# Nadeem202020/VisionTransformer-Intention-Prediction

Hardware: AMD Instinct MI355X
Metric: BEV samples/sec (fwd+bwd) IntentNetViT at 1/2/4/8 MI355X; attn MFMA util % (higher is better)
Workload: dtype bf16

## Files before the change

### visiontransformer-intention-prediction_amd/csrc/attention.hip

```cpp

#include "attn_common.h"

#include <hip/hip_ext.h>

#include <mutex>
#include <vector>

namespace {

constexpr float TAU = 8.0f;

IVIT_DEV float vmax3(float a, float b, float c) {
  float d;
  asm("v_max3_f32 %0, %1, %2, %3" : "=v"(d) : "v"(a), "v"(b), "v"(c));
  return d;
}

struct FwdLdsOff {
  unsigned k[4], v[2][2];
};
IVIT_DEV FwdLdsOff fwd_lds_off(int lane) {
  FwdLdsOff o;
  const int hl = lane >> 5;
#pragma unroll
  for (int ks = 0; ks < 4; ++ks) o.k[ks] = (unsigned)t_off(lane & 31, 2 * ks + hl);
  const int G = lane >> 4, q = (lane >> 2) & 3, p = lane & 3;
#pragma unroll
  for (int cb = 0; cb < 2; ++cb) {
    const int col = 32 * cb + 16 * (G & 1) + 4 * p;
    const int r0 = 4 * (G >> 1) + q, c = col >> 3, e = (col & 7) * 2;
    o.v[cb][0] = (unsigned)(t_off(r0, c) + e);
    o.v[cb][1] = (unsigned)(t_off(r0 + 8, c) + e);
  }
#pragma unroll
  for (int ks = 0; ks < 4; ++ks) asm volatile("" : "+v"(o.k[ks]));
#pragma unroll
  for (int cb = 0; cb < 2; ++cb) asm volatile("" : "+v"(o.v[cb][0]), "+v"(o.v[cb][1]));
  return o;
}

template <bool MASK>
IVIT_DEV float tile_rowmax(f32x16 (&s)[2], int kbase, int N, int lane) {
  const int hl = lane >> 5;
  float a = NEG_BIG, b = NEG_BIG;
#pragma unroll
  for (int t = 0; t < 2; ++t)
#pragma unroll
    for (int r = 0; r < 16; ++r) {
      if (MASK) {
        const int key = kbase + 32 * t + (r & 3) + 8 * (r >> 2) + 4 * hl;
        if (key >= N) s[t][r] = NEG_BIG;
      }
      if (r & 1) b = fmaxf(b, s[t][r]);
      else a = fmaxf(a, s[t][r]);
    }
  return half_swap_max(fmaxf(a, b));
}

IVIT_DEV void qk_tile_c(const char* kimg, const bf16x8 (&qf)[4], const f32x16& init, f32x16 (&s)[2], int lane) {
  const int hl = lane >> 5;
#pragma unroll
  for (int t = 0; t < 2; ++t) {
#pragma unroll
    for (int ks = 0; ks < 4; ++ks) {
      const bf16x8 ka = *(const bf16x8*)(kimg + t_off(32 * t + (lane & 31), 2 * ks + hl));
      s[t] = __builtin_amdgcn_mfma_f32_32x32x16_bf16(ka, qf[ks], ks == 0 ? init : s[t], 0, 0, 0);
    }
  }
}

IVIT_DEV float fwd_step_fenced6(const char* kimg, const char* vimg, const bf16x8 (&qf)[4], const f32x16 (&cur)[2],
                                f32x16 (&nxt)[2], f32x16& o0, f32x16& o1, f32x16& lacc, const bf16x8& ones,
                                const f32x16& negm, int lane, int kbase, int N, const FwdLdsOff& lo) {
  const int hl = lane >> 5;
  auto kfrag = [&](int i) { return *(const bf16x8*)(kimg + lo.k[i & 3] + 4096 * (i >> 2)); };
  unsigned pw[16];
  auto exw = [&](int w) {
    pw[w] = pk_bf16(fast_exp2(cur[(2 * w) >> 4][(2 * w) & 15]), fast_exp2(cur[(2 * w + 1) >> 4][(2 * w + 1) & 15]));
    asm volatile("" : "+v"(pw[w]));
  };
  auto pfrag = [&](int g) {
    return __builtin_bit_cast(bf16x8, make_uint4(pw[4 * g], pw[4 * g + 1], pw[4 * g + 2], pw[4 * g + 3]));
  };
  bf16x8 ka[8];
  ka[0] = kfrag(0);
  ka[1] = kfrag(1);
#pragma unroll
  for (int i = 0; i < 8; ++i) {
    if (i + 2 < 8) ka[i + 2] = kfrag(i + 2);
    const int t = i >> 2, ks = i & 3;
    nxt[t] = __builtin_amdgcn_mfma_f32_32x32x16_bf16(ka[i], qf[ks], ks == 0 ? negm : nxt[t], 0, 0, 0);
    exw(i);
    __builtin_amdgcn_sched_barrier(0);
  }
  bf16x8 vf[8];
  auto vread = [&](int f) {
    union { s16x4 s[2]; bf16x8 v; } u;
    u.s[0] = ds_tr(vimg + lo.v[f & 1][0] + 2048 * (f >> 1));
    u.s[1] = ds_tr(vimg + lo.v[f & 1][1] + 2048 * (f >> 1));
    vf[f] = u.v;
  };
  vread(0);
  vread(1);
  __builtin_amdgcn_sched_barrier(0);
#pragma unroll
  for (int k = 0; k < 6; ++k) {
    const int g = k / 3, which = k % 3;
    if (k == 0) vread(2);
    if (k == 1) vread(3);
    if (k == 3) vread(4);
    if (k == 4) vread(5);
    if (which == 0) o0 = __builtin_amdgcn_mfma_f32_32x32x16_bf16(vf[2 * g], pfrag(g), o0, 0, 0, 0);
    else if (which == 1) o1 = __builtin_amdgcn_mfma_f32_32x32x16_bf16(vf[2 * g + 1], pfrag(g), o1, 0, 0, 0);
    else lacc = __builtin_amdgcn_mfma_f32_32x32x16_bf16(ones, pfrag(g), lacc, 0, 0, 0);
    exw(8 + k);
    __builtin_amdgcn_sched_barrier(0);
  }
  float a = NEG_BIG, bm = NEG_BIG;
  if (kbase + AK > N) {
#pragma unroll
    for (int t = 0; t < 2; ++t)
#pragma unroll
      for (int r = 0; r < 16; ++r) {
        const int key = kbase + 32 * t + (r & 3) + 8 * (r >> 2) + 4 * hl;
        nxt[t][r] = key >= N ? NEG_BIG : nxt[t][r];
      }
  }
#pragma unroll
  for (int k = 6; k < 12; ++k) {
    const int g = k / 3, which = k % 3;
    if (k == 6) vread(6);
    if (k == 7) vread(7);
    if (which == 0) o0 = __builtin_amdgcn_mfma_f32_32x32x16_bf16(vf[2 * g], pfrag(g), o0, 0, 0, 0);
    else if (which == 1) o1 = __builtin_amdgcn_mfma_f32_32x32x16_bf16(vf[2 * g + 1], pfrag(g), o1, 0, 0, 0);
    else lacc = __builtin_amdgcn_mfma_f32_32x32x16_bf16(ones, pfrag(g), lacc, 0, 0, 0);
    if (k == 6) exw(14);
    if (k == 7) exw(15);
    const int v0 = 6 * (k - 6);
#pragma unroll
    for (int v = v0; v < v0 + 6 && v < 32; v += 2) {
      if ((v >> 1) & 1) bm = vmax3(bm, nxt[v >> 4][v & 15], nxt[v >> 4][(v & 15) + 1]);
      else a = vmax3(a, nxt[v >> 4][v & 15], nxt[v >> 4][(v & 15) + 1]);
    }
    __builtin_amdgcn_sched_barrier(0);
  }
  return half_swap_max(fmaxf(a, bm));
}

template <int W, bool PRE>
__global__ __launch_bounds__(64 * W, 8 / W) void attn_fwd_bf16_v6_kernel(const bf16* __restrict__ qkv, int N, int H,
                                                                        bf16* __restrict__ out,
                                                                        float* __restrict__ lse, float c2) {
  __shared__ __attribute__((aligned(16))) char smem[2][2][8192];
  const int tid = threadIdx.x, lane = tid & 63, hl = lane >> 5;
  const int wv = __builtin_amdgcn_readfirstlane(tid >> 6);
  const int2 bid = attn_block_id();
  const int z = bid.y, b = z / H, h = z - b * H;
  const int D = H * 64;
  const long ld = 3L * D;
  const bf16* Qb = qkv + (long)b * N * ld + h * 64;
  const bf16* Kb = Qb + D;
  const bf16* Vb = Qb + 2 * D;
  const int q = bid.x * (32 * W) + wv * 32 + (lane & 31);
  bf16x8 qf[4];
  load_row_frags(Qb + (long)q * ld, q < N, lane, qf);
  if constexpr (PRE) {
#pragma unroll
    for (int i = 0; i < 4; ++i)
#pragma unroll
      for (int e = 0; e < 8; ++e) qf[i][e] = (bf16)((float)qf[i][e] * c2);
  }
  const int nt = (N + AK - 1) / AK, nfull = N / AK;
  unsigned off[8 / W];
#pragma unroll
  for (int i = 0; i < 8 / W; ++i) off[i] = 2u * dma_off<W>(i, wv, lane, ld);
  auto issue1 = [&](const bf16* base, int kt, char* img) {
    const char* sb = uniform_ptr(base + (long)kt * AK * ld);
#pragma unroll
    for (int i = 0; i < 8 / W; ++i) {
      const int piece = wv * (8 / W) + i;
      unsigned o = off[i];
      if (kt >= nfull) {
        const int row = piece * 8 + (lane >> 3), c = (lane & 7) ^ swz128(row);
        o = 2u * (unsigned)((min(kt * AK + row, N - 1) - kt * AK) * ld + c * 8);
      }
      glds_s<false>(o, sb, img + piece * 1024);
    }
  };
  bf16x8 ones;
#pragma unroll
  for (int j = 0; j < 8; ++j) ones[j] = (bf16)1.0f;

  issue1(Kb, 0, smem[0][0]);
  issue1(Vb, 0, smem[0][1]);
  asm volatile("s_waitcnt vmcnt(0)" ::: "memory");
  __builtin_amdgcn_s_barrier();
  if (nt > 1) issue1(Kb, 1, smem[1][0]);
  if (bid.x * (32 * W) + wv * 32 >= N) {
    for (int j = 0; j < nt; ++j) {
      asm volatile("s_waitcnt vmcnt(0)" ::: "memory");
      __builtin_amdgcn_s_barrier();
      if (j + 2 < nt) issue1(Kb, j + 2, smem[j & 1][0]);
      if (j + 1 < nt) issue1(Vb, j + 1, smem[(j & 1) ^ 1][1]);
    }
    return;
  }
  f32x16 sc[2], sn[2];
  qk_tile_c(smem[0][0], qf, zero16(), sc, lane);
  float m = nfull > 0 ? tile_rowmax<false>(sc, 0, N, lane) : tile_rowmax<true>(sc, 0, N, lane);
#pragma unroll
  for (int t = 0; t < 2; ++t)
#pragma unroll
    for (int r = 0; r < 16; ++r) sc[t][r] -= m;
  f32x16 negm;
#pragma unroll
  for (int r = 0; r < 16; ++r) negm[r] = -m;
  f32x16 o0 = zero16(), o1 = zero16(), lacc = zero16();
  const FwdLdsOff lo = fwd_lds_off(lane);

  auto rescale = [&](float mt, f32x16(&nxt)[2]) {
    const bool moved = mt > TAU;
    if (__any(moved)) {
      const float d = moved ? mt : 0.f;
      const float alpha = fast_exp2(-d);
#pragma unroll
      for (int r = 0; r < 16; ++r) { o0[r] *= alpha; o1[r] *= alpha; }
      lacc[0] *= alpha;
#pragma unroll
      for (int t = 0; t < 2; ++t)
#pragma unroll
        for (int r = 0; r < 16; ++r) nxt[t][r] -= d;
      m += d;
#pragma unroll
      for (int r = 0; r < 16; ++r) asm volatile("v_sub_f32 %0, %0, %1" : "+v"(negm[r]) : "v"(d));
    }
  };
  auto body = [&](auto stage, int j, f32x16(&cur)[2], f32x16(&nxt)[2]) {
    constexpr int S = decltype(stage)::value;
    asm volatile("s_waitcnt vmcnt(0)" ::: "memory");
    __builtin_amdgcn_s_barrier();
    if (j + 2 < nt) issue1(Kb, j + 2, smem[S][0]);
    if (j + 1 < nt) issue1(Vb, j + 1, smem[S ^ 1][1]);
    rescale(fwd_step_fenced6(smem[S ^ 1][0], smem[S][1], qf, cur, nxt, o0, o1, lacc, ones, negm, lane,
                               (j + 1) * AK, N, lo),
              nxt);
  };
  using I0 = std::integral_constant<int, 0>;
  using I1 = std::integral_constant<int, 1>;
  int j = 0;
  for (; j + 1 < nt; j += 2) {
    body(I0{}, j, sc, sn);
    body(I1{}, j + 1, sn, sc);
  }
  if (j < nt) body(I0{}, j, sc, sn);
  const float l = lacc[0];
  const float inv = 1.f / l;
  bf16* orow = out + ((long)b * N + (q < N ? q : 0)) * D + h * 64;
  auto emit = [&](const f32x16& o, int dbase) {
#pragma unroll
    for (int g = 0; g < 4; g += 2) {
      const unsigned e0 = pk_bf16(o[4 * g] * inv, o[4 * g + 1] * inv);
      const unsigned e1 = pk_bf16(o[4 * g + 2] * inv, o[4 * g + 3] * inv);
      const unsigned d0 = pk_bf16(o[4 * g + 4] * inv, o[4 * g + 5] * inv);
      const unsigned d1 = pk_bf16(o[4 * g + 6] * inv, o[4 * g + 7] * inv);
      const auto s0 = __builtin_amdgcn_permlane32_swap(d0, e0, false, false);
      const auto s1 = __builtin_amdgcn_permlane32_swap(d1, e1, false, false);
      if (q < N) *(uint4*)(orow + dbase + 8 * (hl ? g : g + 1)) = make_uint4(s0[0], s1[0], s0[1], s1[1]);
    }
  };
  emit(o0, 0);
  emit(o1, 32);
  if (q < N && hl == 0) lse[(long)z * N + q] = (m + log2f(l)) * 0.69314718055994531f;
}

__global__ void attn_prescale_q_kernel(const bf16* __restrict__ qkv, long rows, int D, float c2,
                                       bf16* __restrict__ q2) {
  const long t = (long)blockIdx.x * blockDim.x + threadIdx.x;
  const int cpr = D / 8;
  if (t >= rows * cpr) return;
  const long r = t / cpr;
  const int c = (int)(t - r * cpr) * 8;
  Pack8 x;
  x.u = *(const uint4*)(qkv + r * 3 * D + c);
#pragma unroll
  for (int e = 0; e < 8; ++e) x.h[e] = (bf16)((float)x.h[e] * c2);
  *(uint4*)(q2 + r * D + c) = x.u;
}


constexpr int BNS = 3;

template <int W>
__global__ __launch_bounds__(64 * W, 8 / W) void attn_bwd_dkv_v4_kernel(const bf16* __restrict__ qkv,
                                                                 const bf16* __restrict__ dout,
                                                                 const float* __restrict__ nlse2p,
                                                                 const float* __restrict__ ndeltap, int N, int Npad,
                                                                 int H, bf16* __restrict__ dqkv, float scale,
                                                                 const bf16* __restrict__ qsrc, int ldq) {
  __shared__ __attribute__((aligned(16))) char smem[BNS][2][8192];
  __shared__ __attribute__((aligned(16))) float srow[BNS][2][AK];
  const int tid = threadIdx.x, lane = tid & 63;
  const int g = lane >> 4, c16 = lane & 15;
  const int wv = __builtin_amdgcn_readfirstlane(tid >> 6);
  const int2 bid = attn_block_id();
  const int z = bid.y, b = z / H, h = z - b * H;
  const int D = H * 64;
  const long ld = 3L * D;
  const bf16* Kb = qkv + (long)b * N * ld + D + h * 64;
  const bf16* Vb = Kb + D;
  const bf16* Qb = qsrc + (long)b * N * ldq + h * 64;
  const bf16* Gb = dout + (long)b * N * D + h * 64;
  const char* Ls = uniform_ptr(nlse2p + (long)z * Npad);
  const char* Ds = uniform_ptr(ndeltap + (long)z * Npad);
  constexpr int PW = 8 / W;
  const int kw = bid.x * (32 * W) + wv * 32;
  bf16x8 kf[2][2], vf[2][2];
#pragma unroll
  for (int j = 0; j < 2; ++j) {
    const int key = kw + 16 * j + c16;
#pragma unroll
    for (int s = 0; s < 2; ++s) {
      Pack8 pk, pv;
      pk.u = key < N ? *(const uint4*)(Kb + (long)key * ld + 32 * s + 8 * g) : make_uint4(0, 0, 0, 0);
      pv.u = key < N ? *(const uint4*)(Vb + (long)key * ld + 32 * s + 8 * g) : make_uint4(0, 0, 0, 0);
      kf[j][s] = pk.v;
      vf[j][s] = pv.v;
    }
  }
#pragma unroll
  for (int j = 0; j < 2; ++j) asm volatile("" ::"v"(kf[j][0]), "v"(kf[j][1]), "v"(vf[j][0]), "v"(vf[j][1]));
  f32x4 dk[2][4], dv[2][4];
#pragma unroll
  for (int j = 0; j < 2; ++j)
#pragma unroll
    for (int e = 0; e < 4; ++e) dk[j][e] = dv[j][e] = f32x4{0.f, 0.f, 0.f, 0.f};
  const int nt = (N + AK - 1) / AK, nfull = N / AK;
  unsigned offq[PW], offg[PW];
#pragma unroll
  for (int i = 0; i < PW; ++i) {
    offq[i] = 2u * dma_off16<W>(i, wv, lane, ldq);
    offg[i] = 2u * dma_off16<W>(i, wv, lane, D);
  }
  auto issue = [&](int qt, int S) {
    char* qimg = smem[S][0];
    char* gimg = smem[S][1];
    const char* qb = uniform_ptr(Qb + (long)qt * AK * ldq);
    const char* gb = uniform_ptr(Gb + (long)qt * AK * D);
#pragma unroll
    for (int i = 0; i < PW; ++i) {
      const int piece = wv * PW + i;
      unsigned oq = offq[i], og = offg[i];
      if (qt >= nfull) {
        const int row = piece * 8 + (lane >> 3), c = (lane & 7) ^ (row & 6);
        const int r = min(qt * AK + row, N - 1) - qt * AK;
        oq = 2u * (unsigned)(r * ldq + c * 8);
        og = 2u * (unsigned)(r * D + c * 8);
      }
      glds_s<false>(oq, qb, qimg + piece * 1024);
      glds_s<false>(og, gb, gimg + piece * 1024);
    }
    if (wv == 0) {
      glds4_s(4u * (lane + qt * AK), Ls, &srow[S][0][0]);
      glds4_s(4u * (lane + qt * AK), Ds, &srow[S][1][0]);
    }
  };
  unsigned ro[2], tro[4];
#pragma unroll
  for (int s = 0; s < 2; ++s) ro[s] = (unsigned)t16_off(c16, 4 * s + g);
  {
    const int q = (lane >> 2) & 3, p = lane & 3;
#pragma unroll
    for (int e = 0; e < 4; ++e) tro[e] = (unsigned)(t16_off(4 * g + q, 2 * e + (p >> 1)) + 8 * (p & 1));
  }
#pragma unroll
  for (int s = 0; s < 2; ++s) asm volatile("" : "+v"(ro[s]));
#pragma unroll
  for (int e = 0; e < 4; ++e) asm volatile("" : "+v"(tro[e]));

  bf16x8 qa[2][2], ga[2][2];
  f32x4 sn[2], dn[2];
  bf16x8 tg[4], tq[4];
  auto read_frag = [&](const char* qimg, const char* gimg, int t, int i, int s) {
    qa[i][s] = *(const bf16x8*)(qimg + ro[s] + 4096 * t + 2048 * i);
    ga[i][s] = *(const bf16x8*)(gimg + ro[s] + 4096 * t + 2048 * i);
  };
  auto read_rows = [&](const float* lr, const float* dr, int t, int i) {
    sn[i] = *(const f32x4*)(lr + 32 * t + 16 * i + 4 * g);
    dn[i] = *(const f32x4*)(dr + 32 * t + 16 * i + 4 * g);
  };
  auto word8 = [&](const unsigned (&w)[4]) { return __builtin_bit_cast(bf16x8, make_uint4(w[0], w[1], w[2], w[3])); };
  auto read_b = [&](const char* qimg, const char* gimg, int t, int e) {
    union { s16x4 s[2]; bf16x8 v; } a, c;
    a.s[0] = ds_tr(gimg + tro[e] + 4096 * t);
    a.s[1] = ds_tr(gimg + tro[e] + 4096 * t + 2048);
    c.s[0] = ds_tr(qimg + tro[e] + 4096 * t);
    c.s[1] = ds_tr(qimg + tro[e] + 4096 * t + 2048);
    tg[e] = a.v;
    tq[e] = c.v;
  };
  float ep0, ep1, et0, et1;
  auto e_sub = [&](const f32x4& S, const f32x4& DP, int hh, int ph, unsigned& wu, unsigned& wd) {
    if (ph == 0) {
      ep0 = fast_exp2(S[2 * hh]);
      asm volatile("" : "+v"(ep0));
    }
    if (ph == 1) {
      ep1 = fast_exp2(S[2 * hh + 1]);
      asm volatile("" : "+v"(ep1));
    }
    if (ph == 2) {
      et0 = ep0 * DP[2 * hh];
      et1 = ep1 * DP[2 * hh + 1];
      asm volatile("" : "+v"(et0), "+v"(et1));
    }
    if (ph == 3) {
      wu = pk_bf16(ep0, ep1);
      wd = pk_bf16(et0, et1);
      asm volatile("" : "+v"(wu), "+v"(wd));
    }
  };
  f32x4 sc1[2], dc1[2];
  unsigned upA[4], udA[4];
  unsigned up1[4], ud1[4];
  auto body = [&](auto sa, auto ta, auto sb, auto tb, auto sn_, auto tn, auto bar, int jn, bool more) {
    constexpr int SA = decltype(sa)::value, TA = decltype(ta)::value, SB = decltype(sb)::value;
    constexpr int TB = decltype(tb)::value, SN = decltype(sn_)::value, TN = decltype(tn)::value;
    constexpr bool BAR = decltype(bar)::value;
    f32x4 s[2][2], dp[2][2];
    unsigned upN[4], udN[4];
#pragma unroll
    for (int m = 0; m < 16; ++m) {
      const int ks = m >> 3, i = (m >> 2) & 1, j = (m >> 1) & 1;
      if ((m & 1) == 0) s[i][j] = mfma16(qa[i][ks], kf[j][ks], ks == 0 ? sn[i] : s[i][j]);
      else dp[i][j] = mfma16(ga[i][ks], vf[j][ks], ks == 0 ? dn[i] : dp[i][j]);
      if (m == 0) read_frag(smem[SA][0], smem[SA][1], TA, 0, 1);
      if (m == 2) read_frag(smem[SA][0], smem[SA][1], TA, 1, 1);
      {
        const int q = m >> 2, ie = q >> 1, hh = q & 1;
        e_sub(sc1[ie], dc1[ie], hh, m & 3, up1[2 * ie + hh], ud1[2 * ie + hh]);
      }
      if (m == 9) read_b(smem[SB][0], smem[SB][1], TB, 0);
      if (m == 12) read_b(smem[SB][0], smem[SB][1], TB, 1);
      __builtin_amdgcn_sched_barrier(0);
    }
    if constexpr (BAR) {
      asm volatile("s_waitcnt vmcnt(0)" ::: "memory");
      __builtin_amdgcn_s_barrier();
      if (jn < nt) issue(jn, jn % BNS);
    }
#pragma unroll
    for (int m = 0; m < 16; ++m) {
      const int e = m >> 2, j = (m >> 1) & 1;
      if (m == 0) read_b(smem[SB][0], smem[SB][1], TB, 2);
      if (m == 2) read_b(smem[SB][0], smem[SB][1], TB, 3);
      if ((m & 1) == 0) dv[j][e] = mfma16(word8(j ? up1 : upA), tg[e], dv[j][e]);
      else dk[j][e] = mfma16(word8(j ? ud1 : udA), tq[e], dk[j][e]);
      {
        const int q = m >> 2, ie = q >> 1, hh = q & 1;
        e_sub(s[ie][0], dp[ie][0], hh, m & 3, upN[2 * ie + hh], udN[2 * ie + hh]);
      }
      if (more) {
        if (m == 5) read_rows(srow[SN][0], srow[SN][1], TN, 0);
        if (m == 7) read_rows(srow[SN][0], srow[SN][1], TN, 1);
        if (m == 9) read_frag(smem[SN][0], smem[SN][1], TN, 0, 0);
        if (m == 11) read_frag(smem[SN][0], smem[SN][1], TN, 1, 0);
      }
      __builtin_amdgcn_sched_barrier(0);
    }
#pragma unroll
    for (int i = 0; i < 2; ++i) {
      sc1[i] = s[i][1];
      dc1[i] = dp[i][1];
    }
#pragma unroll
    for (int w = 0; w < 4; ++w) {
      upA[w] = upN[w];
      udA[w] = udN[w];
    }
  };
  using I0 = std::integral_constant<int, 0>;
  using I1 = std::integral_constant<int, 1>;
  using I2 = std::integral_constant<int, 2>;
  using F = std::false_type;
  using T = std::true_type;

  issue(0, 0);
  if (nt > 1) issue(1, 1);
  {
    uint4* z2 = (uint4*)&smem[2][0][0];
    for (int i = tid; i < 2 * 8192 / 16; i += 64 * W) z2[i] = make_uint4(0, 0, 0, 0);
  }
  asm volatile("s_waitcnt vmcnt(0) lgkmcnt(0)" ::: "memory");
  __builtin_amdgcn_s_barrier();
#pragma unroll
  for (int i = 0; i < 2; ++i) {
    read_rows(srow[0][0], srow[0][1], 0, i);
    read_frag(smem[0][0], smem[0][1], 0, i, 0);
  }
#pragma unroll
  for (int i = 0; i < 2; ++i) {
    sc1[i] = f32x4{NEG_BIG, NEG_BIG, NEG_BIG, NEG_BIG};
    dc1[i] = f32x4{0.f, 0.f, 0.f, 0.f};
  }
#pragma unroll
  for (int w = 0; w < 4; ++w) upA[w] = udA[w] = 0u;
  if (kw >= N) {
    for (int j = 0; j < nt; ++j) {
      asm volatile("s_waitcnt vmcnt(0)" ::: "memory");
      __builtin_amdgcn_s_barrier();
      if (j + 2 < nt) issue(j + 2, (j + 2) % BNS);
    }
    __syncthreads();
    return;
  }
  auto tile = [&](auto st, int j) {
    constexpr int S = decltype(st)::value;
    using SP = std::integral_constant<int, (S + BNS - 1) % BNS>;
    using SNX = std::integral_constant<int, (S + 1) % BNS>;
    using SC = std::integral_constant<int, S>;
    body(SC{}, I0{}, SP{}, I1{}, SC{}, I1{}, F{}, 0, true);
    body(SC{}, I1{}, SC{}, I0{}, SNX{}, I0{}, T{}, j + 2, j + 1 < nt);
  };
  int j = 0;
  for (; j + 3 <= nt; j += 3) {
    tile(I0{}, j);
    tile(I1{}, j + 1);
    tile(I2{}, j + 2);
  }
  if (j < nt) tile(I0{}, j);
  if (j + 1 < nt) tile(I1{}, j + 1);
  {
    const int S = (nt - 1) % BNS;
#pragma unroll
    for (int q = 0; q < 4; ++q)
#pragma unroll
      for (int ph = 0; ph < 4; ++ph) e_sub(sc1[q >> 1], dc1[q >> 1], q & 1, ph, up1[q], ud1[q]);
#pragma unroll
    for (int e = 0; e < 4; ++e) read_b(smem[S][0], smem[S][1], 1, e);
#pragma unroll
    for (int e = 0; e < 4; ++e) {
      dv[0][e] = mfma16(word8(upA), tg[e], dv[0][e]);
      dk[0][e] = mfma16(word8(udA), tq[e], dk[0][e]);
      dv[1][e] = mfma16(word8(up1), tg[e], dv[1][e]);
      dk[1][e] = mfma16(word8(ud1), tq[e], dk[1][e]);
    }
  }
  __syncthreads();
  char* tl = &smem[0][0][0] + wv * 2 * 4608;
  bf16* base = dqkv + (long)b * N * ld + h * 64;
  wave_tile_store(tl, dk, scale, base + D, ld, kw, N, lane);
  wave_tile_store(tl + 4608, dv, 1.0f, base + 2 * D, ld, kw, N, lane);
}

IVIT_DEV void dq16_tile_masked(const char* kimg, const char* vimg, const bf16x8 (&qf)[2][2], const bf16x8 (&gf)[2][2],
                               const f32x4 (&nl)[2], const f32x4 (&nd)[2], f32x4 (&dq)[2][4], int kbase, int N,
                               int lane) {
  const int g = lane >> 4, c16 = lane & 15, q = (lane >> 2) & 3, p = lane & 3;
#pragma unroll
  for (int t = 0; t < 2; ++t) {
    if (kbase + 32 * t >= N) break;
    f32x4 s[2][2], dp[2][2];
#pragma unroll
    for (int j = 0; j < 2; ++j)
#pragma unroll
      for (int i = 0; i < 2; ++i) {
        s[j][i] = nl[i];
        dp[j][i] = nd[i];
#pragma unroll
        for (int ks = 0; ks < 2; ++ks) {
          const bf16x8 ka = *(const bf16x8*)(kimg + t16_off(32 * t + 16 * j + c16, 4 * ks + g));
          const bf16x8 va = *(const bf16x8*)(vimg + t16_off(32 * t + 16 * j + c16, 4 * ks + g));
          s[j][i] = mfma16(ka, qf[i][ks], s[j][i]);
          dp[j][i] = mfma16(va, gf[i][ks], dp[j][i]);
        }
      }
    unsigned w[2][4];
#pragma unroll
    for (int i = 0; i < 2; ++i)
#pragma unroll
      for (int j = 0; j < 2; ++j)
#pragma unroll
        for (int hh = 0; hh < 2; ++hh) {
          float d0 = fast_exp2(s[j][i][2 * hh]) * dp[j][i][2 * hh];
          float d1 = fast_exp2(s[j][i][2 * hh + 1]) * dp[j][i][2 * hh + 1];
          const int key = kbase + 32 * t + 16 * j + 4 * g + 2 * hh;
          if (key >= N) d0 = 0.f;
          if (key + 1 >= N) d1 = 0.f;
          w[i][2 * j + hh] = pk_bf16(d0, d1);
        }
#pragma unroll
    for (int e = 0; e < 4; ++e) {
      const int off = t16_off(32 * t + 4 * g + q, 2 * e + (p >> 1)) + 8 * (p & 1);
      union { s16x4 s[2]; bf16x8 v; } u;
      u.s[0] = ds_tr(kimg + off);
      u.s[1] = ds_tr(kimg + off + 2048);
#pragma unroll
      for (int i = 0; i < 2; ++i)
        dq[i][e] = mfma16(__builtin_bit_cast(bf16x8, make_uint4(w[i][0], w[i][1], w[i][2], w[i][3])), u.v, dq[i][e]);
    }
  }
}

template <int W>
__global__ __launch_bounds__(64 * W, 8 / W) void attn_bwd_dq_v4_kernel(const bf16* __restrict__ qkv,
                                                                const bf16* __restrict__ dout,
                                                                float* __restrict__ nlse2p,
                                                                float* __restrict__ ndeltap, int N, int Npad, int H,
                                                                bf16* __restrict__ dqkv, float scale,
                                                                const bf16* __restrict__ out,
                                                                const float* __restrict__ lse,
                                                                const bf16* __restrict__ qsrc, int ldq) {
  __shared__ __attribute__((aligned(16))) char smem[BNS][2][8192];
  const int tid = threadIdx.x, lane = tid & 63;
  const int g = lane >> 4, c16 = lane & 15;
  const int wv = __builtin_amdgcn_readfirstlane(tid >> 6);
  const int2 bid = attn_block_id();
  const int z = bid.y, b = z / H, h = z - b * H;
  const int D = H * 64;
  const long ld = 3L * D;
  const bf16* Kb = qkv + (long)b * N * ld + D + h * 64;
  const bf16* Vb = Kb + D;
  const bf16* Qb = qsrc + (long)b * N * ldq + h * 64;
  constexpr int PW = 8 / W;
  const int qw = bid.x * (32 * W) + wv * 32;
  bf16x8 qf[2][2], gf[2][2];
  f32x4 nl[2], nd[2];
#pragma unroll
  for (int i = 0; i < 2; ++i) {
    const int q = qw + 16 * i + c16;
    const bool qv = q < N;
    bf16x8 of[2];
#pragma unroll
    for (int s = 0; s < 2; ++s) {
      Pack8 pq, pg, po;
      const long orow = ((long)b * N + q) * D + h * 64 + 32 * s + 8 * g;
      pq.u = qv ? *(const uint4*)(Qb + (long)q * ldq + 32 * s + 8 * g) : make_uint4(0, 0, 0, 0);
      pg.u = qv ? *(const uint4*)(dout + orow) : make_uint4(0, 0, 0, 0);
      po.u = qv ? *(const uint4*)(out + orow) : make_uint4(0, 0, 0, 0);
      qf[i][s] = pq.v;
      gf[i][s] = pg.v;
      of[s] = po.v;
    }
    float d = 0.f;
#pragma unroll
    for (int s = 0; s < 2; ++s)
#pragma unroll
      for (int e = 0; e < 8; ++e) d = fmaf((float)of[s][e], (float)gf[i][s][e], d);
    d += __shfl_xor(d, 16, 64);
    d += __shfl_xor(d, 32, 64);
    const float lse2 = qv ? lse[(long)z * N + q] * LOG2E : 1e30f;
    const float dlt = qv ? d : 0.f;
    if (g == 0 && q < Npad) {
      nlse2p[(long)z * Npad + q] = -lse2;
      ndeltap[(long)z * Npad + q] = -dlt;
    }
    nl[i] = f32x4{-lse2, -lse2, -lse2, -lse2};
    nd[i] = f32x4{-dlt, -dlt, -dlt, -dlt};
  }
  f32x4 dq[2][4];
#pragma unroll
  for (int i = 0; i < 2; ++i)
#pragma unroll
    for (int e = 0; e < 4; ++e) dq[i][e] = f32x4{0.f, 0.f, 0.f, 0.f};
  const int nt = (N + AK - 1) / AK, nfull = N / AK;
  unsigned off[PW];
#pragma unroll
  for (int i = 0; i < PW; ++i) off[i] = 2u * dma_off16<W>(i, wv, lane, ld);
  auto issue = [&](int kt, int S) {
    char* kimg = smem[S][0];
    char* vimg = smem[S][1];
    const char* kb = uniform_ptr(Kb + (long)kt * AK * ld);
    const char* vb = uniform_ptr(Vb + (long)kt * AK * ld);
#pragma unroll
    for (int i = 0; i < PW; ++i) {
      const int piece = wv * PW + i;
      unsigned o = off[i];
      if (kt >= nfull) {
        const int row = piece * 8 + (lane >> 3), c = (lane & 7) ^ (row & 6);
        o = 2u * (unsigned)((min(kt * AK + row, N - 1) - kt * AK) * ld + c * 8);
      }
      glds_s<false>(o, kb, kimg + piece * 1024);
      glds_s<false>(o, vb, vimg + piece * 1024);
    }
  };
  issue(0, 0);
  if (nt > 1) issue(1, 1);
  {
    uint4* z2 = (uint4*)&smem[2][0][0];
    for (int i = tid; i < 2 * 8192 / 16; i += 64 * W) z2[i] = make_uint4(0, 0, 0, 0);
  }
  asm volatile("s_waitcnt vmcnt(0) lgkmcnt(0)" ::: "memory");
  __builtin_amdgcn_s_barrier();

  if (qw >= N) {
    for (int j = 0; j < nfull; ++j) {
      asm volatile("s_waitcnt vmcnt(0)" ::: "memory");
      __builtin_amdgcn_s_barrier();
      if (j + 2 < nt) issue(j + 2, (j + 2) % BNS);
    }
    if (nt > nfull) {
      asm volatile("s_waitcnt vmcnt(0)" ::: "memory");
      __builtin_amdgcn_s_barrier();
    }
    __syncthreads();
    return;
  }
  if (nfull > 0) {
    unsigned ro[2], tro[4];
#pragma unroll
    for (int s = 0; s < 2; ++s) ro[s] = (unsigned)t16_off(c16, 4 * s + g);
    {
      const int q = (lane >> 2) & 3, p = lane & 3;
#pragma unroll
      for (int e = 0; e < 4; ++e) tro[e] = (unsigned)(t16_off(4 * g + q, 2 * e + (p >> 1)) + 8 * (p & 1));
    }
#pragma unroll
    for (int s = 0; s < 2; ++s) asm volatile("" : "+v"(ro[s]));
#pragma unroll
    for (int e = 0; e < 4; ++e) asm volatile("" : "+v"(tro[e]));
    bf16x8 ka[2][2], va[2][2];
    bf16x8 tk[4];
    auto read_a = [&](const char* kimg, const char* vimg, int t, int j, int ks) {
      ka[j][ks] = *(const bf16x8*)(kimg + ro[ks] + 4096 * t + 2048 * j);
      va[j][ks] = *(const bf16x8*)(vimg + ro[ks] + 4096 * t + 2048 * j);
    };
    auto read_b = [&](const char* kimg, int t, int e) {
      union { s16x4 s[2]; bf16x8 v; } u;
      u.s[0] = ds_tr(kimg + tro[e] + 4096 * t);
      u.s[1] = ds_tr(kimg + tro[e] + 4096 * t + 2048);
      tk[e] = u.v;
    };
    auto word8 = [&](const unsigned (&w)[4]) { return __builtin_bit_cast(bf16x8, make_uint4(w[0], w[1], w[2], w[3])); };
    float ep0, ep1, et0, et1;
    auto e_sub = [&](const f32x4& S, const f32x4& DP, int hh, int ph, unsigned& w) {
      if (ph == 0) {
        ep0 = fast_exp2(S[2 * hh]);
        asm volatile("" : "+v"(ep0));
      }
      if (ph == 1) {
        ep1 = fast_exp2(S[2 * hh + 1]);
        asm volatile("" : "+v"(ep1));
      }
      if (ph == 2) {
        et0 = ep0 * DP[2 * hh];
        et1 = ep1 * DP[2 * hh + 1];
        asm volatile("" : "+v"(et0), "+v"(et1));
      }
      if (ph == 3) {
        w = pk_bf16(et0, et1);
        asm volatile("" : "+v"(w));
      }
    };
    f32x4 sc1[2], dc1[2];
    unsigned pdqA[4];
    unsigned pdq1[4];
    auto body = [&](auto sa, auto ta, auto sb, auto tb, auto sn_, auto tn, auto bar, int jn, bool more) {
      constexpr int SA = decltype(sa)::value, TA = decltype(ta)::value, SB = decltype(sb)::value;
      constexpr int TB = decltype(tb)::value, SN = decltype(sn_)::value, TN = decltype(tn)::value;
      constexpr bool BAR = decltype(bar)::value;
      f32x4 s[2][2], dp[2][2];
      unsigned pdqN[4];
#pragma unroll
      for (int m = 0; m < 16; ++m) {
        const int ks = m >> 3, j = (m >> 2) & 1, i = (m >> 1) & 1;
        if ((m & 1) == 0) s[j][i] = mfma16(ka[j][ks], qf[i][ks], ks == 0 ? nl[i] : s[j][i]);
        else dp[j][i] = mfma16(va[j][ks], gf[i][ks], ks == 0 ? nd[i] : dp[j][i]);
        if (m == 0) read_a(smem[SA][0], smem[SA][1], TA, 0, 1);
        if (m == 2) read_a(smem[SA][0], smem[SA][1], TA, 1, 1);
        {
          const int q = m >> 2, je = q >> 1, hh = q & 1;
          e_sub(sc1[je], dc1[je], hh, m & 3, pdq1[2 * je + hh]);
        }
        if (m == 8) read_b(smem[SB][0], TB, 0);
        if (m == 10) read_b(smem[SB][0], TB, 1);
        if (m == 12) read_b(smem[SB][0], TB, 2);
        if (m == 14) read_b(smem[SB][0], TB, 3);
        __builtin_amdgcn_sched_barrier(0);
      }
      if constexpr (BAR) {
        asm volatile("s_waitcnt vmcnt(0)" ::: "memory");
        __builtin_amdgcn_s_barrier();
        if (jn < nt) issue(jn, jn % BNS);
      }
#pragma unroll
      for (int m = 0; m < 8; ++m) {
        const int e = m >> 1, i = m & 1;
        dq[i][e] = mfma16(word8(i ? pdq1 : pdqA), tk[e], dq[i][e]);
        {
          const int q = m >> 1, je = q >> 1, hh = q & 1;
          e_sub(s[je][0], dp[je][0], hh, 2 * (m & 1), pdqN[2 * je + hh]);
          e_sub(s[je][0], dp[je][0], hh, 2 * (m & 1) + 1, pdqN[2 * je + hh]);
        }
        if (more) {
          if (m == 1) read_a(smem[SN][0], smem[SN][1], TN, 0, 0);
          if (m == 3) read_a(smem[SN][0], smem[SN][1], TN, 1, 0);
        }
        __builtin_amdgcn_sched_barrier(0);
      }
#pragma unroll
      for (int j = 0; j < 2; ++j) {
        sc1[j] = s[j][1];
        dc1[j] = dp[j][1];
      }
#pragma unroll
      for (int w = 0; w < 4; ++w) pdqA[w] = pdqN[w];
    };
    using I0 = std::integral_constant<int, 0>;
    using I1 = std::integral_constant<int, 1>;
    using I2 = std::integral_constant<int, 2>;
    using F = std::false_type;
    using T = std::true_type;
#pragma unroll
    for (int j = 0; j < 2; ++j) read_a(smem[0][0], smem[0][1], 0, j, 0);
#pragma unroll
    for (int j = 0; j < 2; ++j) {
      sc1[j] = f32x4{NEG_BIG, NEG_BIG, NEG_BIG, NEG_BIG};
      dc1[j] = f32x4{0.f, 0.f, 0.f, 0.f};
    }
#pragma unroll
    for (int w = 0; w < 4; ++w) pdqA[w] = 0u;
    auto tile = [&](auto st, int j) {
      constexpr int S = decltype(st)::value;
      using SP = std::integral_constant<int, (S + BNS - 1) % BNS>;
      using SNX = std::integral_constant<int, (S + 1) % BNS>;
      using SC = std::integral_constant<int, S>;
      body(SC{}, I0{}, SP{}, I1{}, SC{}, I1{}, F{}, 0, true);
      body(SC{}, I1{}, SC{}, I0{}, SNX{}, I0{}, T{}, j + 2, j + 1 < nfull);
    };
    int j = 0;
    for (; j + 3 <= nfull; j += 3) {
      tile(I0{}, j);
      tile(I1{}, j + 1);
      tile(I2{}, j + 2);
    }
    if (j < nfull) tile(I0{}, j);
    if (j + 1 < nfull) tile(I1{}, j + 1);
    {
      const int S = (nfull - 1) % BNS;
#pragma unroll
      for (int q = 0; q < 4; ++q)
#pragma unroll
        for (int ph = 0; ph < 4; ++ph) e_sub(sc1[q >> 1], dc1[q >> 1], q & 1, ph, pdq1[q]);
#pragma unroll
      for (int e = 0; e < 4; ++e) read_b(smem[S][0], 1, e);
#pragma unroll
      for (int e = 0; e < 4; ++e) {
        dq[0][e] = mfma16(word8(pdqA), tk[e], dq[0][e]);
        dq[1][e] = mfma16(word8(pdq1), tk[e], dq[1][e]);
      }
    }
  }
  if (nt > nfull) {
    asm volatile("s_waitcnt vmcnt(0)" ::: "memory");
    __builtin_amdgcn_s_barrier();
    const int S = nfull % BNS;
    dq16_tile_masked(smem[S][0], smem[S][1], qf, gf, nl, nd, dq, nfull * AK, N, lane);
  }
  __syncthreads();
  wave_tile_store(&smem[0][0][0] + wv * 4608, dq, scale, dqkv + (long)b * N * ld + h * 64, ld, qw, N, lane);
}

__global__ void softmax_rows_kernel(float* __restrict__ S, long ldS, int N, float* __restrict__ lse) {
  const long row = blockIdx.x;
  float* s = S + row * ldS;
  __shared__ float red[4];
  float mx = -INFINITY;
  for (int i = threadIdx.x; i < N; i += 256) mx = fmaxf(mx, s[i]);
  mx = wave_max(mx);
  if ((threadIdx.x & 63) == 0) red[threadIdx.x >> 6] = mx;
  __syncthreads();
  mx = fmaxf(fmaxf(red[0], red[1]), fmaxf(red[2], red[3]));
  __syncthreads();
  float sum = 0.f;
  for (int i = threadIdx.x; i < N; i += 256) {
    const float e = expf(s[i] - mx);
    s[i] = e;
    sum += e;
  }
  sum = wave_sum(sum);
  if ((threadIdx.x & 63) == 0) red[threadIdx.x >> 6] = sum;
  __syncthreads();
  sum = red[0] + red[1] + red[2] + red[3];
  const float inv = 1.f / sum;
  for (int i = threadIdx.x; i < ldS; i += 256) s[i] = i < N ? s[i] * inv : 0.f;
  if (threadIdx.x == 0) lse[row] = mx + logf(sum);
}

__global__ void prob_rows_kernel(float* __restrict__ S, long ldS, int N, const float* __restrict__ lse) {
  const long row = blockIdx.x;
  float* s = S + row * ldS;
  const float l = lse[row];
  for (int i = threadIdx.x; i < ldS; i += 256) s[i] = i < N ? expf(s[i] - l) : 0.f;
}

__global__ void dsoftmax_rows_kernel(const float* __restrict__ P, float* __restrict__ dP, long ldS, int N) {
  const long row = blockIdx.x;
  const float* p = P + row * ldS;
  float* g = dP + row * ldS;
  __shared__ float red[4];
  float s = 0.f;
  for (int i = threadIdx.x; i < N; i += 256) s += p[i] * g[i];
  s = wave_sum(s);
  if ((threadIdx.x & 63) == 0) red[threadIdx.x >> 6] = s;
  __syncthreads();
  s = red[0] + red[1] + red[2] + red[3];
  for (int i = threadIdx.x; i < ldS; i += 256) g[i] = i < N ? p[i] * (g[i] - s) : 0.f;
}

long ld_scores(long N) { return (N + 7) / 8 * 8; }

}

namespace {
struct KtRec {
  int tag;
  hipEvent_t start, stop;
};
std::mutex kt_mu;
bool kt_on = false;
std::vector<KtRec> kt_recs;
std::vector<hipEvent_t> kt_pool;
size_t kt_used = 0;

hipEvent_t kt_event() {
  if (kt_used == kt_pool.size()) {
    hipEvent_t e = nullptr;
    if (hipEventCreate(&e) != hipSuccess) return nullptr;
    kt_pool.push_back(e);
  }
  return kt_pool[kt_used++];
}

template <typename K, typename... Args>
void kt_launch(int tag, K kernel, dim3 g, dim3 b, hipStream_t st, Args... args) {
  hipEvent_t e0 = nullptr, e1 = nullptr;
  {
    std::lock_guard<std::mutex> lk(kt_mu);
    if (kt_on) {
      e0 = kt_event();
      e1 = e0 ? kt_event() : nullptr;
      if (e0 && e1) kt_recs.push_back({tag, e0, e1});
    }
  }
  if (e0 && e1)
    hipExtLaunchKernelGGL(kernel, g, b, 0, st, e0, e1, 0, args...);
  else
    hipLaunchKernelGGL(kernel, g, b, 0, st, args...);
}
}


namespace {
void attn_bwd_v4_launch(const void* qkv, const void* out, const void* dout, const float* lse, long B, long N, long H,
                        void* dqkv, float* nlse2p, const void* qsrc, int ldq, hipStream_t st) {
  const float scale = 0.125f;
  const long Npad = (N + AK - 1) / AK * AK;
  float* ndeltap = nlse2p + B * H * Npad;
  constexpr int BW = 4;
  const dim3 gw(ivit_cdiv(N, 32 * BW), B * H);
  kt_launch(IVIT_KT_ATTN_BWD_DQ, attn_bwd_dq_v4_kernel<BW>, gw, dim3(64 * BW), st, (const bf16*)qkv,
            (const bf16*)dout, nlse2p, ndeltap, (int)N, (int)Npad, (int)H, (bf16*)dqkv, scale, (const bf16*)out, lse,
            (const bf16*)qsrc, ldq);
  kt_launch(IVIT_KT_ATTN_BWD_DKV, attn_bwd_dkv_v4_kernel<BW>, gw, dim3(64 * BW), st, (const bf16*)qkv,
            (const bf16*)dout, nlse2p, ndeltap, (int)N, (int)Npad, (int)H, (bf16*)dqkv, 0.69314718055994531f,
            (const bf16*)qsrc, ldq);
}
}

static long attn_rows_bytes(long B, long N, long H) { return 2 * B * H * ((N + AK - 1) / AK * AK) * 4; }

extern "C" long ivit_attn_workspace(int dtype, long B, long N, long H, long Dh, int backward) {
  if (dtype == IVIT_BF16) return backward ? attn_rows_bytes(B, N, H) + B * N * H * Dh * 2 : 0;
  const long one = B * H * N * ld_scores(N) * 4;
  return backward ? 2 * one : one;
}

extern "C" int ivit_attn_fwd(int dtype, const void* qkv, long B, long N, long H, long Dh, void* out, float* lse,
                             void* work, long work_bytes, void* stream) {
  IVIT_CHECK_ARG(Dh == 64, "ivit_attn_fwd: head dim must be 64 (got %ld)", Dh);
  IVIT_CHECK_ARG(work_bytes >= ivit_attn_workspace(dtype, B, N, H, Dh, 0), "ivit_attn_fwd: workspace too small");
  hipStream_t st = ivit_stream(stream);
  const float scale = 1.0f / sqrtf((float)Dh);
  if (B * N * H == 0) return 0;
  if (dtype == IVIT_BF16) {
    dim3 g(ivit_cdiv(N, 128), B * H);
    hipLaunchKernelGGL((attn_fwd_bf16_v6_kernel<4, true>), g, dim3(256), 0, st, (const bf16*)qkv, (int)N, (int)H,
                       (bf16*)out, lse, scale * LOG2E);
    IVIT_LAUNCH_CHECK();
    return 0;
  }
  const long D = H * Dh, ldq = 3 * D, ldS = ld_scores(N);
  float* S = (float*)work;
  const float* Q = (const float*)qkv;
  LdDense<float> la{Q, ldq, (int)N, (int)Dh, 0, 0, 0, {H, N * ldq, Dh}};
  LdDense<float> lb{Q + D, ldq, (int)N, (int)Dh, 0, 0, 0, {H, N * ldq, Dh}};
  EpiStore<float> es{S, ldS, {1, N * ldS, 0}, nullptr, IVIT_ACT_NONE, nullptr, scale};
  launch_gemm<true, true>(false, la, lb, es, (int)N, (int)N, (int)Dh, (int)(B * H), 1, st);
  hipLaunchKernelGGL(softmax_rows_kernel, dim3(B * H * N), dim3(256), 0, st, S, ldS, (int)N, lse);
  LdDense<float> lp{S, ldS, (int)N, (int)ldS, 0, 0, 0, {1, N * ldS, 0}};
  LdDense<float> lv{Q + 2 * D, ldq, (int)N, (int)Dh, 0, 0, 0, {H, N * ldq, Dh}};
  EpiStore<float> eo{(float*)out, D, {H, N * D, Dh}, nullptr, IVIT_ACT_NONE, nullptr, 1.f};
  launch_gemm<true, false>(false, lp, lv, eo, (int)N, (int)Dh, (int)ldS, (int)(B * H), 1, st);
  IVIT_LAUNCH_CHECK();
  return 0;
}

extern "C" int ivit_attn_bwd(int dtype, const void* qkv, const void* out, const void* dout, const float* lse, long B,
                             long N, long H, long Dh, void* dqkv, void* work, long work_bytes, void* stream) {
  IVIT_CHECK_ARG(Dh == 64, "ivit_attn_bwd: head dim must be 64 (got %ld)", Dh);
  IVIT_CHECK_ARG(work_bytes >= ivit_attn_workspace(dtype, B, N, H, Dh, 1), "ivit_attn_bwd: workspace too small");
  hipStream_t st = ivit_stream(stream);
  const float scale = 1.0f / sqrtf((float)Dh);
  if (B * N * H == 0) return 0;
  const long D = H * Dh, ldq = 3 * D;
  if (dtype == IVIT_BF16) {
    float* nlse2p = (float*)work;
    bf16* q2 = (bf16*)((char*)work + attn_rows_bytes(B, N, H));
    hipLaunchKernelGGL(attn_prescale_q_kernel, dim3(ivit_cdiv(B * N * D / 8, 256)), dim3(256), 0, st,
                       (const bf16*)qkv, B * N, (int)D, scale * LOG2E, q2);
    attn_bwd_v4_launch(qkv, out, dout, lse, B, N, H, dqkv, nlse2p, q2, (int)D, st);
    IVIT_LAUNCH_CHECK();
    return 0;
  }
  const long ldS = ld_scores(N), zs = N * ldS;
  float* P = (float*)work;
  float* dP = P + B * H * zs;
  const float* Q = (const float*)qkv;
  float* dq = (float*)dqkv;
  const int Z = (int)(B * H);
  const BatchOff qoff{H, N * ldq, Dh}, soff{1, zs, 0}, ooff{H, N * D, Dh};
  {
    LdDense<float> la{Q, ldq, (int)N, (int)Dh, 0, 0, 0, qoff};
    LdDense<float> lb{Q + D, ldq, (int)N, (int)Dh, 0, 0, 0, qoff};
    EpiStore<float> es{P, ldS, soff, nullptr, IVIT_ACT_NONE, nullptr, scale};
    launch_gemm<true, true>(false, la, lb, es, (int)N, (int)N, (int)Dh, Z, 1, st);
    hipLaunchKernelGGL(prob_rows_kernel, dim3(Z * N), dim3(256), 0, st, P, ldS, (int)N, lse);
  }
  {
    LdDense<float> la{P, ldS, (int)N, (int)ldS, 0, 0, 0, soff};
    LdDense<float> lb{(const float*)dout, D, (int)N, (int)Dh, 0, 0, 0, ooff};
    EpiStore<float> e{dq + 2 * D, ldq, qoff, nullptr, IVIT_ACT_NONE, nullptr, 1.f};
    launch_gemm<false, false>(false, la, lb, e, (int)N, (int)Dh, (int)N, Z, 1, st);
  }
  {
    LdDense<float> la{(const float*)dout, D, (int)N, (int)Dh, 0, 0, 0, ooff};
    LdDense<float> lb{Q + 2 * D, ldq, (int)N, (int)Dh, 0, 0, 0, qoff};
    EpiStore<float> e{dP, ldS, soff, nullptr, IVIT_ACT_NONE, nullptr, 1.f};
    launch_gemm<true, true>(false, la, lb, e, (int)N, (int)N, (int)Dh, Z, 1, st);
    hipLaunchKernelGGL(dsoftmax_rows_kernel, dim3(Z * N), dim3(256), 0, st, P, dP, ldS, (int)N);
  }
  {
    LdDense<float> la{dP, ldS, (int)N, (int)ldS, 0, 0, 0, soff};
    LdDense<float> lb{Q + D, ldq, (int)N, (int)Dh, 0, 0, 0, qoff};
    EpiStore<float> e{dq, ldq, qoff, nullptr, IVIT_ACT_NONE, nullptr, scale};
    launch_gemm<true, false>(false, la, lb, e, (int)N, (int)Dh, (int)ldS, Z, 1, st);
  }
  {
    LdDense<float> la{dP, ldS, (int)N, (int)ldS, 0, 0, 0, soff};
    LdDense<float> lb{Q, ldq, (int)N, (int)Dh, 0, 0, 0, qoff};
    EpiStore<float> e{dq + D, ldq, qoff, nullptr, IVIT_ACT_NONE, nullptr, scale};
    launch_gemm<false, false>(false, la, lb, e, (int)N, (int)Dh, (int)N, Z, 1, st);
  }
  IVIT_LAUNCH_CHECK();
  return 0;
}

extern "C" int ivit_ktime_arm(int on) {
  std::lock_guard<std::mutex> lk(kt_mu);
  if (on) {
    kt_recs.clear();
    kt_used = 0;
  }
  kt_on = on != 0;
  return 0;
}

extern "C" int ivit_ktime_read(int tag, double* start_ms, double* stop_ms, long cap, long* count) {
  IVIT_CHECK_ARG(tag >= 0 && tag < IVIT_KT_NTAGS, "ivit_ktime_read: unknown tag %d", tag);
  IVIT_CHECK_ARG(count && (cap == 0 || (start_ms && stop_ms)), "ivit_ktime_read: null output");
  std::lock_guard<std::mutex> lk(kt_mu);
  long n = 0;
  for (const KtRec& r : kt_recs) {
    if (r.tag != tag) continue;
    float t0 = 0.f, t1 = 0.f;
    hipError_t e = hipEventSynchronize(r.stop);
    if (e == hipSuccess) e = hipEventElapsedTime(&t0, kt_recs[0].start, r.start);
    if (e == hipSuccess) e = hipEventElapsedTime(&t1, kt_recs[0].start, r.stop);
    if (e != hipSuccess) {
      ivit_set_error("ivit_ktime_read: %s", hipGetErrorString(e));
      return (int)e;
    }
    if (n < cap) {
      start_ms[n] = t0;
      stop_ms[n] = t1;
    }
    ++n;
  }
  *count = n;
  return 0;
}

extern "C" int ivit_attn_fwd_q2(const void* qkv, long B, long N, long H, long Dh, void* out, float* lse, void* work,
                                long work_bytes, void* stream) {
  IVIT_CHECK_ARG(Dh == 64, "ivit_attn_fwd_q2: head dim must be 64 (got %ld)", Dh);
  (void)work;
  (void)work_bytes;
  if (B * N * H == 0) return 0;
  dim3 g(ivit_cdiv(N, 128), B * H);
  kt_launch(IVIT_KT_ATTN_FWD, attn_fwd_bf16_v6_kernel<4, false>, g, dim3(256), ivit_stream(stream), (const bf16*)qkv,
            (int)N, (int)H, (bf16*)out, lse, 1.0f);
  IVIT_LAUNCH_CHECK();
  return 0;
}

extern "C" int ivit_attn_bwd_q2(const void* qkv, const void* out, const void* dout, const float* lse, long B, long N,
                                long H, long Dh, void* dqkv, void* work, long work_bytes, void* stream) {
  IVIT_CHECK_ARG(Dh == 64, "ivit_attn_bwd_q2: head dim must be 64 (got %ld)", Dh);
  IVIT_CHECK_ARG(work_bytes >= attn_rows_bytes(B, N, H), "ivit_attn_bwd_q2: workspace too small");
  if (B * N * H == 0) return 0;
  attn_bwd_v4_launch(qkv, out, dout, lse, B, N, H, dqkv, (float*)work, qkv, (int)(3 * H * Dh), ivit_stream(stream));
  IVIT_LAUNCH_CHECK();
  return 0;
}
```

Before: 185.5.

## Stage Q fragments in LDS and reorder QK/PV interleave to raise occupancy

Q fragments are no longer kept in registers for the whole kernel. Each wave writes its Q into a per-wave LDS image, either by direct global-to-LDS DMA or a scaled store, and re-reads the fragments from LDS on every QK step. The softmax max is recovered from negm instead of a separate m register, and the launch bounds rise from 8/W to 12/W to target more waves per SIMD. The QK and PV MFMA loops are reinterleaved so that half the QK work overlaps the first PV group. The trade-off is extra LDS reads and LDS footprint in exchange for lower VGPR pressure and better latency hiding.

```diff
diff --git a/visiontransformer-intention-prediction_amd/csrc/attention.hip b/visiontransformer-intention-prediction_amd/csrc/attention.hip
--- a/visiontransformer-intention-prediction_amd/csrc/attention.hip
+++ b/visiontransformer-intention-prediction_amd/csrc/attention.hip
@@ -17,10 +17,12 @@
 }
 
 struct FwdLdsOff {
-  unsigned k[4], v[2][2];
+  unsigned k[4], v[2][2], q;
 };
-IVIT_DEV FwdLdsOff fwd_lds_off(int lane) {
+IVIT_DEV FwdLdsOff fwd_lds_off(int lane, int wv) {
   FwdLdsOff o;
+  o.q = (unsigned)(4096 * wv + 16 * lane);
+  asm volatile("" : "+v"(o.q));
   const int hl = lane >> 5;
 #pragma unroll
   for (int ks = 0; ks < 4; ++ks) o.k[ks] = (unsigned)t_off(lane & 31, 2 * ks + hl);
@@ -69,7 +71,7 @@
   }
 }
 
-IVIT_DEV float fwd_step_fenced6(const char* kimg, const char* vimg, const bf16x8 (&qf)[4], const f32x16 (&cur)[2],
+IVIT_DEV float fwd_step_fenced6(const char* kimg, const char* vimg, const char* qimg, const f32x16 (&cur)[2],
                                 f32x16 (&nxt)[2], f32x16& o0, f32x16& o1, f32x16& lacc, const bf16x8& ones,
                                 const f32x16& negm, int lane, int kbase, int N, const FwdLdsOff& lo) {
   const int hl = lane >> 5;
@@ -82,41 +84,71 @@
   auto pfrag = [&](int g) {
     return __builtin_bit_cast(bf16x8, make_uint4(pw[4 * g], pw[4 * g + 1], pw[4 * g + 2], pw[4 * g + 3]));
   };
-  bf16x8 ka[8];
-  ka[0] = kfrag(0);
-  ka[1] = kfrag(1);
-#pragma unroll
-  for (int i = 0; i < 8; ++i) {
-    if (i + 2 < 8) ka[i + 2] = kfrag(i + 2);
-    const int t = i >> 2, ks = i & 3;
-    nxt[t] = __builtin_amdgcn_mfma_f32_32x32x16_bf16(ka[i], qf[ks], ks == 0 ? negm : nxt[t], 0, 0, 0);
-    exw(i);
-    __builtin_amdgcn_sched_barrier(0);
-  }
-  bf16x8 vf[8];
+  bf16x8 ka[8], qf[8], vf[8];
+  unsigned qo = lo.q;
+  auto qfrag = [&](int i) {
+    if (i == 4) asm volatile("" : "+v"(qo));
+    return *(const bf16x8*)(qimg + qo + 1024 * (i & 3));
+  };
+  auto kq = [&](int i) {
+    ka[i] = kfrag(i);
+    qf[i] = qfrag(i);
+  };
   auto vread = [&](int f) {
     union { s16x4 s[2]; bf16x8 v; } u;
     u.s[0] = ds_tr(vimg + lo.v[f & 1][0] + 2048 * (f >> 1));
     u.s[1] = ds_tr(vimg + lo.v[f & 1][1] + 2048 * (f >> 1));
     vf[f] = u.v;
   };
-  vread(0);
-  vread(1);
-  __builtin_amdgcn_sched_barrier(0);
-#pragma unroll
-  for (int k = 0; k < 6; ++k) {
+  auto qk = [&](int i) {
+    const int t = i >> 2, ks = i & 3;
+    nxt[t] = __builtin_amdgcn_mfma_f32_32x32x16_bf16(ka[i], qf[i], ks == 0 ? negm : nxt[t], 0, 0, 0);
+  };
+  auto pv = [&](int k) {
     const int g = k / 3, which = k % 3;
-    if (k == 0) vread(2);
-    if (k == 1) vread(3);
-    if (k == 3) vread(4);
-    if (k == 4) vread(5);
     if (which == 0) o0 = __builtin_amdgcn_mfma_f32_32x32x16_bf16(vf[2 * g], pfrag(g), o0, 0, 0, 0);
     else if (which == 1) o1 = __builtin_amdgcn_mfma_f32_32x32x16_bf16(vf[2 * g + 1], pfrag(g), o1, 0, 0, 0);
     else lacc = __builtin_amdgcn_mfma_f32_32x32x16_bf16(ones, pfrag(g), lacc, 0, 0, 0);
-    exw(8 + k);
+  };
+  float a = NEG_BIG, bm = NEG_BIG;
+  auto rmax = [&](int v0, int n) {
+#pragma unroll
+    for (int v = 2 * v0; v < 2 * (v0 + n); v += 2) {
+      if ((v >> 1) & 1) bm = vmax3(bm, nxt[v >> 4][v & 15], nxt[v >> 4][(v & 15) + 1]);
+      else a = vmax3(a, nxt[v >> 4][v & 15], nxt[v >> 4][(v & 15) + 1]);
+    }
+  };
+  kq(0);
+  kq(1);
+#pragma unroll
+  for (int i = 0; i < 4; ++i) {
+    if (i + 2 < 4) kq(i + 2);
+    if (i == 2) vread(0);
+    if (i == 3) vread(1);
+    qk(i);
+    exw(i);
     __builtin_amdgcn_sched_barrier(0);
   }
-  float a = NEG_BIG, bm = NEG_BIG;
+#pragma unroll
+  for (int k = 0; k < 6; ++k) {
+    if (k == 0) vread(2);
+    if (k == 1) vread(3);
+    if (k == 4) kq(4);
+    if (k == 5) kq(5);
+    pv(k);
+    exw(4 + k + (k > 2));
+    if (k == 2) exw(7);
+    __builtin_amdgcn_sched_barrier(0);
+  }
+#pragma unroll
+  for (int i = 4; i < 8; ++i) {
+    if (i + 2 < 8) kq(i + 2);
+    if (i == 6) vread(4);
+    if (i == 7) vread(5);
+    qk(i);
+    exw(7 + i);
+    __builtin_amdgcn_sched_barrier(0);
+  }
   if (kbase + AK > N) {
 #pragma unroll
     for (int t = 0; t < 2; ++t)
@@ -128,30 +160,24 @@
   }
 #pragma unroll
   for (int k = 6; k < 12; ++k) {
-    const int g = k / 3, which = k % 3;
     if (k == 6) vread(6);
     if (k == 7) vread(7);
-    if (which == 0) o0 = __builtin_amdgcn_mfma_f32_32x32x16_bf16(vf[2 * g], pfrag(g), o0, 0, 0, 0);
-    else if (which == 1) o1 = __builtin_amdgcn_mfma_f32_32x32x16_bf16(vf[2 * g + 1], pfrag(g), o1, 0, 0, 0);
-    else lacc = __builtin_amdgcn_mfma_f32_32x32x16_bf16(ones, pfrag(g), lacc, 0, 0, 0);
-    if (k == 6) exw(14);
-    if (k == 7) exw(15);
-    const int v0 = 6 * (k - 6);
-#pragma unroll
-    for (int v = v0; v < v0 + 6 && v < 32; v += 2) {
-      if ((v >> 1) & 1) bm = vmax3(bm, nxt[v >> 4][v & 15], nxt[v >> 4][(v & 15) + 1]);
-      else a = vmax3(a, nxt[v >> 4][v & 15], nxt[v >> 4][(v & 15) + 1]);
-    }
+    pv(k);
+    if (k == 6) exw(15);
+    if (k == 6) rmax(0, 2);
+    else if (k == 11) rmax(14, 2);
+    else rmax(3 * (k - 7) + 2, 3);
     __builtin_amdgcn_sched_barrier(0);
   }
   return half_swap_max(fmaxf(a, bm));
 }
 
 template <int W, bool PRE>
-__global__ __launch_bounds__(64 * W, 8 / W) void attn_fwd_bf16_v6_kernel(const bf16* __restrict__ qkv, int N, int H,
-                                                                        bf16* __restrict__ out,
-                                                                        float* __restrict__ lse, float c2) {
+__global__ __launch_bounds__(64 * W, 12 / W) void attn_fwd_bf16_v6_kernel(const bf16* __restrict__ qkv, int N, int H,
+                                                                         bf16* __restrict__ out,
+                                                                         float* __restrict__ lse, float c2) {
   __shared__ __attribute__((aligned(16))) char smem[2][2][8192];
+  __shared__ __attribute__((aligned(16))) char qimg[W][4][1024];
   const int tid = threadIdx.x, lane = tid & 63, hl = lane >> 5;
   const int wv = __builtin_amdgcn_readfirstlane(tid >> 6);
   const int2 bid = attn_block_id();
@@ -162,13 +188,23 @@
   const bf16* Kb = Qb + D;
   const bf16* Vb = Qb + 2 * D;
   const int q = bid.x * (32 * W) + wv * 32 + (lane & 31);
-  bf16x8 qf[4];
-  load_row_frags(Qb + (long)q * ld, q < N, lane, qf);
-  if constexpr (PRE) {
-#pragma unroll
-    for (int i = 0; i < 4; ++i)
-#pragma unroll
-      for (int e = 0; e < 8; ++e) qf[i][e] = (bf16)((float)qf[i][e] * c2);
+  {
+    const int q0 = bid.x * (32 * W);
+    const int qrow = min(q, N - 1) - q0;
+    if constexpr (PRE) {
+      bf16x8 qf[4];
+      load_row_frags(Qb + (long)(q0 + qrow) * ld, true, lane, qf);
+#pragma unroll
+      for (int i = 0; i < 4; ++i) {
+#pragma unroll
+        for (int e = 0; e < 8; ++e) qf[i][e] = (bf16)((float)qf[i][e] * c2);
+        *(bf16x8*)(qimg[wv][i] + 16 * lane) = qf[i];
+      }
+    } else {
+      const char* sb = uniform_ptr(Qb + (long)q0 * ld);
+#pragma unroll
+      for (int i = 0; i < 4; ++i) glds_s<false>(2u * (unsigned)(qrow * ld + 16 * i + 8 * hl), sb, qimg[wv][i]);
+    }
   }
   const int nt = (N + AK - 1) / AK, nfull = N / AK;
   unsigned off[8 / W];
@@ -205,9 +241,15 @@
     }
     return;
   }
+  const FwdLdsOff lo = fwd_lds_off(lane, wv);
   f32x16 sc[2], sn[2];
-  qk_tile_c(smem[0][0], qf, zero16(), sc, lane);
-  float m = nfull > 0 ? tile_rowmax<false>(sc, 0, N, lane) : tile_rowmax<true>(sc, 0, N, lane);
+  {
+    bf16x8 qf[4];
+#pragma unroll
+    for (int i = 0; i < 4; ++i) qf[i] = *(const bf16x8*)(&qimg[0][0][0] + lo.q + 1024 * i);
+    qk_tile_c(smem[0][0], qf, zero16(), sc, lane);
+  }
+  const float m = nfull > 0 ? tile_rowmax<false>(sc, 0, N, lane) : tile_rowmax<true>(sc, 0, N, lane);
 #pragma unroll
   for (int t = 0; t < 2; ++t)
 #pragma unroll
@@ -216,7 +258,6 @@
 #pragma unroll
   for (int r = 0; r < 16; ++r) negm[r] = -m;
   f32x16 o0 = zero16(), o1 = zero16(), lacc = zero16();
-  const FwdLdsOff lo = fwd_lds_off(lane);
 
   auto rescale = [&](float mt, f32x16(&nxt)[2]) {
     const bool moved = mt > TAU;
@@ -230,7 +271,6 @@
       for (int t = 0; t < 2; ++t)
 #pragma unroll
         for (int r = 0; r < 16; ++r) nxt[t][r] -= d;
-      m += d;
 #pragma unroll
       for (int r = 0; r < 16; ++r) asm volatile("v_sub_f32 %0, %0, %1" : "+v"(negm[r]) : "v"(d));
     }
@@ -241,7 +281,7 @@
     __builtin_amdgcn_s_barrier();
     if (j + 2 < nt) issue1(Kb, j + 2, smem[S][0]);
     if (j + 1 < nt) issue1(Vb, j + 1, smem[S ^ 1][1]);
-    rescale(fwd_step_fenced6(smem[S ^ 1][0], smem[S][1], qf, cur, nxt, o0, o1, lacc, ones, negm, lane,
+    rescale(fwd_step_fenced6(smem[S ^ 1][0], smem[S][1], &qimg[0][0][0], cur, nxt, o0, o1, lacc, ones, negm, lane,
                                (j + 1) * AK, N, lo),
               nxt);
   };
@@ -270,7 +310,7 @@
   };
   emit(o0, 0);
   emit(o1, 32);
-  if (q < N && hl == 0) lse[(long)z * N + q] = (m + log2f(l)) * 0.69314718055994531f;
+  if (q < N && hl == 0) lse[(long)z * N + q] = (log2f(l) - negm[0]) * 0.69314718055994531f;
 }
 
 __global__ void attn_prescale_q_kernel(const bf16* __restrict__ qkv, long rows, int D, float c2,
```

Measured after the change: 186.7, median of 6. No clear change (+0.7%).
